# bjo5029/causal-vae

Measured on AMD Instinct MI355X. Metric: training samples/sec on 128^3 vessel volumes (3D CausalVAE train step), higher is better.
Workload: dtype bf16; 1 GPU; 3D vessel CausalVAE train step, 128^3 bf16 volumes (z-scored N(0,1)), batch 4/GPU, Adam lr 0.0001, ELBO = MSE-sum + 2000*MSE-sum(m) + KLD; global_batch=4, per_gpu_batch=4, parallelism=dp1, params=15346957

## Files before the change

causal_vae_amd/_lib.py:

```python
import ctypes as C
import os

import torch

_HERE = os.path.dirname(os.path.abspath(__file__))
LIB_PATH = os.environ.get("CVAE_HIP_LIB") or os.path.join(_HERE, "libcvae_hip.so")

F32, BF16, FP8 = 0, 1, 2
ACT_NONE, ACT_RELU, ACT_SIGMOID, ACT_LEAKY02, ACT_LEAKY001 = 0, 1, 2, 3, 4
_ACT = {None: ACT_NONE, "none": ACT_NONE, "relu": ACT_RELU, "sigmoid": ACT_SIGMOID, "leaky02": ACT_LEAKY02, "leaky001": ACT_LEAKY001}


class CvaeError(RuntimeError):
    pass


if not os.path.exists(LIB_PATH):
    raise ImportError(
        f"{LIB_PATH} is missing: build it with `python -c 'import __graft_entry__ as g; g.build()'` "
        "(or `make -C causal_vae_amd/csrc`).  causal_vae_amd has no CPU / eager fallback.")
lib = C.CDLL(LIB_PATH)

_p, _i64, _i, _f, _sz, _u64 = C.c_void_p, C.c_int64, C.c_int, C.c_float, C.c_size_t, C.c_uint64

# ... 70 lines not shown
    "cvae_softmax_ce_bwd": [_p, _p, _p, _p, _i64, _i64, _p],
    "cvae_uniform_kl_fwd": [_p, _p, _i64, _i64, _p, _sz, _p],
    "cvae_uniform_kl_bwd": [_p, _p, _p, _i64, _i64, _p],
    "cvae_adam_step": [_p, _p, _p, _p, _i64, _f, _f, _f, _f, _f, _f, _p, _p],
    "cvae_adam_multi": [_p, _p, _p, _p, _p, _i, _f, _f, _f, _f, _f, _f, _p, _p, _p],
    "cvae_multi_copy": [_p, _p, _p, _i, _p],
    "cvae_counter_add": [_p, _i, _p],
    "cvae_sqnorm": [_p, _p, _i64, _p, _sz, _p],
    "cvae_sqnorm_multi": [_p, _p, _i, _p, _p, _sz, _p],
    "cvae_weighted_sum": [_p, _p, _i, _p, _p, _i, _p],
    "cvae_scale": [_p, _i64, _p, _p],
    "cvae_clip_coef": [_p, _p, _f, _p],
    "cvae_up2x_supported": [_i64] * 7,
    "cvae_up2x_fwd": [_p, _p] + [_i64] * 7 + [_i, _p],
    "cvae_elbo_up2x_partials": [_i64] * 4,
    "cvae_elbo_up2x_fwd": [_p] * 6 + [_f, _p, _p, _p, _p, _p] + [_i64] * 9 + [_i, _p],
    "cvae_elbo_up2x_bwd": [_p] * 5 + [_f] + [_p] * 5 + [_i64] * 9 + [_i, _p],
    "cvae_conv3_to_k4": [_p, _p, _i64, _i64, _p],
    "cvae_k4_to_conv3_grad": [_p, _p, _i64, _i64, _p],
    "cvae_clamp_fwd": [_p, _p, _f, _f, _i64, _p],
    "cvae_clamp_bwd": [_p, _p, _p, _f, _f, _i64, _p],
    "cvae_bn2d_workspace_bytes": [_i64, _i64],
    "cvae_bn2d_fwd": [_p] * 8 + [_i64, _i64, _f, _f, _i, _i, _i, _p, _sz, _p],
    "cvae_bn2d_bwd": [_p] * 9 + [_i64, _i64, _i, _i, _p, _sz, _p],
    "cvae_fold_bn_conv": [_i] + [_p] * 11 + [_p],
    "cvae_fold_bn_conv_bwd": [_i] + [_p] * 14 + [_p],
    "cvae_vit_tokens": [_p, _i, _p, _p, _p, _i64, _i64, _p],
    "cvae_layernorm256": [_p, _i64, _p, _p, _p, _i64, _f, _i, _p],
    "cvae_token_gemm": [_p, _i64, _p, _p, _p, _i64, _p, _i64, _i64, _i64, _i64, _i, _i, _p],
    "cvae_mhsa_fwd": [_p] * 4 + [_i64] * 9 + [_i, _p],
    "cvae_mhsa_fwd_train": [_p] * 5 + [_i64] * 9 + [_i, _p],
# ... 154 lines not shown
```

causal_vae_amd/csrc/recon_loss.hip:

```cpp
#include "common.h"

namespace {

__device__ __forceinline__ void load4_f32(const float* p, float* o) { const float4 v = *(const float4*)p; o[0] = v.x; o[1] = v.y; o[2] = v.z; o[3] = v.w; }
__device__ __forceinline__ void load4_f32(const bf16* p, float* o) {
    const uint2 v = *(const uint2*)p;
    o[0] = __uint_as_float(v.x << 16); o[1] = __uint_as_float(v.x & 0xffff0000u); o[2] = __uint_as_float(v.y << 16); o[3] = __uint_as_float(v.y & 0xffff0000u);
}

CVAE_TUNABLE(UP2X_STREAM_BYTES, 256 << 20);

__device__ __forceinline__ float2 even_w(int o) { return o == 0 ? make_float2(0.f, 1.f) : make_float2(0.25f, 0.75f); }

#define CVAE_ELBO_TICKET_GROUPS 32
struct ElboFinish {
    unsigned* ticket;
    const float *m_hat, *m, *mu, *logvar;
    float* out4;
    int* bump;
    float gamma;
    int n_m, n_z;
};
struct SmallBwd {
    const float *m_hat, *m, *mu, *logvar;
    float *d_mhat, *dmu, *dlv;
    float gamma;
    int n_m, n_z, main_blocks;
};
template <typename T, int MODE>
__global__ __launch_bounds__(256) void up2x_block_kernel(const T* __restrict__ src, const float* __restrict__ xin, float* __restrict__ dst,
                                                         float* __restrict__ acc_out, const float* __restrict__ gout, float gscale,
                                                         int B, int d, int h, int w, int D, int H, int W, SmallBwd sb, ElboFinish fin) {
    constexpr int J0 = (MODE == 3) ? -1 : 0, NJ = (MODE == 3) ? 10 : 8;
    const bool sdz = D != d;
    const float sw = (float)w / (float)W;
    const int wg = w >> 2, n = B * d * h * wg;
    const int i0 = blockIdx.x * 256 + threadIdx.x, lane = threadIdx.x & 63;
    const bool live = i0 < n;
    const int i = live ? i0 : n - 1;
    float sse = 0.f;
    {
        int r = i;
        const int xg = r % wg; r /= wg;
        const int y = r % h; r /= h;
        const int z = r % d;
        const int b = r / d;
        const int x0 = 4 * xg, ow0 = 8 * xg;
        float4 xa_[2][2], xb_[2][2];
        float xl_[2][2], xr_[2][2];
        if (MODE == 1 || MODE == 3) {
#pragma unroll
            for (int a = 0; a < 2; ++a)
#pragma unroll
                for (int bq = 0; bq < 2; ++bq) {
                    const int od = sdz ? 2 * z + a : z, oh = 2 * y + bq;
                    const size_t rowoff = ((size_t)(b * D + od) * H + oh) * W;
                    xa_[a][bq] = *(const float4*)(xin + rowoff + ow0);
                    xb_[a][bq] = *(const float4*)(xin + rowoff + ow0 + 4);
                    if (MODE == 3) {
                        const float el = xin[rowoff + max(ow0 - 1, 0)], er = xin[rowoff + min(ow0 + 8, W - 1)];
                        const float lft = __shfl_up(xb_[a][bq].w, 1), rgt = __shfl_down(xa_[a][bq].x, 1);
                        xl_[a][bq] = (ow0 > 0) ? (lane > 0 ? lft : el) : 0.f;
                        xr_[a][bq] = (ow0 + 8 < W) ? (lane < 63 ? rgt : er) : 0.f;
                    }
                }
        }
        float P[3][3][NJ];
        const float2 ew0 = even_w(ow0);
#pragma unroll
        for (int zr = 0; zr < 3; ++zr) {
            const int zi = sdz ? min(max(z - 1 + zr, 0), d - 1) : z;
#pragma unroll
            for (int yr = 0; yr < 3; ++yr) {
                const int yi = min(max(y - 1 + yr, 0), h - 1);
                const T* row = src + ((size_t)(b * d + zi) * h + yi) * w;
                float v[6];
                load4_f32(row + x0, v + 1);
                const float el = to_f32(row[max(x0 - 1, 0)]), er = to_f32(row[min(x0 + 4, w - 1)]);
                const float lft = __shfl_up(v[4], 1), rgt = __shfl_down(v[1], 1);
                v[0] = (xg == 0) ? v[1] : (lane > 0 ? lft : el);
                v[5] = (xg == wg - 1) ? v[4] : (lane < 63 ? rgt : er);
#pragma unroll
                for (int j = 0; j < NJ; ++j) {
                    const int jj = J0 + j;
                    if (jj & 1) {
                        const int c = (jj + 1) / 2;
                        P[zr][yr][j] = 0.75f * v[c] + 0.25f * v[c + 1];
                    } else {
                        const int c = jj / 2;
                        const float2 ww = (jj == 0) ? ew0 : make_float2(0.25f, 0.75f);
                        P[zr][yr][j] = ww.x * v[c] + ww.y * v[c + 1];
                    }
                }
            }
        }
        Win4 wx[4];
        if (MODE == 3) {
#pragma unroll
            for (int q = 0; q < 4; ++q) wx[q] = win4<int>(x0 + q, w, W, sw, true);
        }
#pragma unroll
        for (int a = 0; a < 2; ++a) {
            if (!live || (!sdz && a == 1)) break;
            const int od = sdz ? 2 * z + a : z;
            const int zr0 = a;
            const float2 dw = !sdz ? make_float2(1.f, 0.f) : (a == 0 ? even_w(od) : make_float2(0.75f, 0.25f));
#pragma unroll
            for (int bq = 0; bq < 2; ++bq) {
                const int oh = 2 * y + bq;
                const float2 hw = (bq == 0) ? even_w(oh) : make_float2(0.75f, 0.25f);
                float o[NJ];
#pragma unroll
                for (int j = 0; j < NJ; ++j) {
                    const float lo = hw.x * P[zr0][bq][j] + hw.y * P[zr0][bq + 1][j];
                    const float hi = hw.x * P[zr0 + 1][bq][j] + hw.y * P[zr0 + 1][bq + 1][j];
                    o[j] = dw.x * lo + dw.y * hi;
                }
                const size_t rowoff = ((size_t)(b * D + od) * H + oh) * W;
                if (MODE == 0 || MODE == 4) {
                    const f32x4 oa = {o[0], o[1], o[2], o[3]}, ob = {o[4], o[5], o[6], o[7]};
                    if (MODE == 4) {
                        __builtin_nontemporal_store(oa, (f32x4*)(dst + rowoff + ow0));
                        __builtin_nontemporal_store(ob, (f32x4*)(dst + rowoff + ow0 + 4));
                    } else {
                        *(f32x4*)(dst + rowoff + ow0) = oa;
                        *(f32x4*)(dst + rowoff + ow0 + 4) = ob;
                    }
                } else {
                    const float4 xa = xa_[a][bq], xb = xb_[a][bq];
                    const float xv[8] = {xa.x, xa.y, xa.z, xa.w, xb.x, xb.y, xb.z, xb.w};
                    if (MODE == 1) {
#pragma unroll
                        for (int j = 0; j < 8; ++j) { const float df = o[j] - xv[j]; sse += df * df; }
                    } else {
                        float g[10];
                        g[0] = (ow0 > 0) ? o[0] - xl_[a][bq] : 0.f;
#pragma unroll
                        for (int j = 0; j < 8; ++j) { g[1 + j] = o[1 + j] - xv[j]; sse += g[1 + j] * g[1 + j]; }
                        g[9] = (ow0 + 8 < W) ? o[9] - xr_[a][bq] : 0.f;
                        float t1v[4];
#pragma unroll
                        for (int q = 0; q < 4; ++q) {
                            float rs = 0.f;
#pragma unroll
                            for (int c = 0; c < 4; ++c) if (wx[q].w[c] != 0.f) rs += wx[q].w[c] * g[2 * q + c];
                            t1v[q] = rs;
                        }
                        *(float4*)(dst + ((size_t)(b * D + od) * H + oh) * w + x0) = make_float4(t1v[0], t1v[1], t1v[2], t1v[3]);
                    }
                }
            }
        }
    }
    if (MODE == 1 || MODE == 3) {
        __shared__ float red[4];
        __shared__ unsigned is_last;
        sse = wave_sum(sse);
        if ((threadIdx.x & 63) == 0) red[threadIdx.x >> 6] = sse;
        __syncthreads();
        if (!fin.ticket) {
            if (threadIdx.x == 0) acc_out[blockIdx.x] = red[0] + red[1] + red[2] + red[3];
            return;
        }
        if (threadIdx.x == 0) {
            __hip_atomic_store(acc_out + blockIdx.x, red[0] + red[1] + red[2] + red[3], __ATOMIC_RELAXED, __HIP_MEMORY_SCOPE_AGENT);
            asm volatile("s_waitcnt vmcnt(0)" ::: "memory");
            constexpr unsigned G = CVAE_ELBO_TICKET_GROUPS;
            const unsigned grp = blockIdx.x % G, pop = gridDim.x / G + (grp < gridDim.x % G ? 1u : 0u), ngrp = gridDim.x < G ? gridDim.x : G;
            unsigned last = 0u;
            if (__hip_atomic_fetch_add(fin.ticket + 32 * grp, 1u, __ATOMIC_RELAXED, __HIP_MEMORY_SCOPE_AGENT) == pop - 1)
                last = __hip_atomic_fetch_add(fin.ticket + 32 * G, 1u, __ATOMIC_RELAXED, __HIP_MEMORY_SCOPE_AGENT) == ngrp - 1 ? 1u : 0u;
            is_last = last;
        }
        __syncthreads();
        if (!is_last) return;
        __shared__ float fr[3][4];
        float sr = 0.f, sm = 0.f, sk = 0.f;
        for (int i0 = threadIdx.x; i0 < (int)gridDim.x; i0 += 256 * 8) {
            float pv[8];
#pragma unroll
            for (int u = 0; u < 8; ++u) pv[u] = (i0 + 256 * u < (int)gridDim.x) ? __hip_atomic_load(acc_out + i0 + 256 * u, __ATOMIC_RELAXED, __HIP_MEMORY_SCOPE_AGENT) : 0.f;
#pragma unroll
            for (int u = 0; u < 8; ++u) if (i0 + 256 * u < (int)gridDim.x) sr += pv[u];
        }
        for (int i = threadIdx.x; i < fin.n_m; i += 256) { const float df = fin.m_hat[i] - fin.m[i]; sm += df * df; }
        for (int i = threadIdx.x; i < fin.n_z; i += 256) sk += 1.f + fin.logvar[i] - fin.mu[i] * fin.mu[i] - expf(fin.logvar[i]);
        sr = wave_sum(sr); sm = wave_sum(sm); sk = wave_sum(sk);
        if ((threadIdx.x & 63) == 0) { fr[0][threadIdx.x >> 6] = sr; fr[1][threadIdx.x >> 6] = sm; fr[2][threadIdx.x >> 6] = sk; }
        __syncthreads();
        if (threadIdx.x == 0) {
            const float recon = fr[0][0] + fr[0][1] + fr[0][2] + fr[0][3], ml = fr[1][0] + fr[1][1] + fr[1][2] + fr[1][3];
            const float kld = -0.5f * (fr[2][0] + fr[2][1] + fr[2][2] + fr[2][3]);
            fin.out4[0] = recon + fin.gamma * ml + kld; fin.out4[1] = recon; fin.out4[2] = ml; fin.out4[3] = kld;
            if (fin.bump) *fin.bump += 1;
        }
        if (threadIdx.x <= CVAE_ELBO_TICKET_GROUPS) __hip_atomic_store(fin.ticket + 32 * threadIdx.x, 0u, __ATOMIC_RELAXED, __HIP_MEMORY_SCOPE_AGENT);
    }
}

template <typename T, bool NT>
__global__ __launch_bounds__(256) void up2x_tile_kernel(const T* __restrict__ src, float* __restrict__ dst, int d, int h, int w) {
    constexpr int TZ = 2, TY = 8, TX = 64, PZ = TZ + 2, PY = TY + 2, PITCH = TX + 4;
    constexpr int VEC = 16 / sizeof(T), SEGS = TX / VEC;
    __shared__ __attribute__((aligned(16))) float tile[PZ * PY * PITCH];
    const int t = threadIdx.x;
    int blk = blockIdx.x;
    const int xt = blk % (w / TX); blk /= (w / TX);
    const int yt = blk % (h / TY); blk /= (h / TY);
    const int zt = blk % (d / TZ), b = blk / (d / TZ);
    const int x0 = xt * TX, y0 = yt * TY, z0 = zt * TZ;
    const T* sb = src + (size_t)b * d * h * w;
    for (int i = t; i < PZ * PY * SEGS; i += 256) {
// ... 115 lines not shown
    for (int i = threadIdx.x; i < n_z; i += 256) sk += 1.f + logvar[i] - mu[i] * mu[i] - expf(logvar[i]);
    sr = wave_sum(sr); sm = wave_sum(sm); sk = wave_sum(sk);
    if ((threadIdx.x & 63) == 0) { red[0][threadIdx.x >> 6] = sr; red[1][threadIdx.x >> 6] = sm; red[2][threadIdx.x >> 6] = sk; }
    __syncthreads();
    if (threadIdx.x == 0) {
        const float recon = red[0][0] + red[0][1] + red[0][2] + red[0][3], ml = red[1][0] + red[1][1] + red[1][2] + red[1][3];
        const float kld = -0.5f * (red[2][0] + red[2][1] + red[2][2] + red[2][3]);
        out4[0] = recon + gamma * ml + kld; out4[1] = recon; out4[2] = ml; out4[3] = kld;
    }
}

bool up2x_ok(int64_t B, int64_t d, int64_t h, int64_t w, int64_t D, int64_t H, int64_t W) {
    return B > 0 && d > 0 && h > 0 && w > 0 && (D == 2 * d || (D == 1 && d == 1)) && H == 2 * h && W == 2 * w && (w % 4) == 0 && B * D * H * W < (int64_t)1 << 31;
}

}

extern "C" int cvae_up2x_supported(int64_t B, int64_t d, int64_t h, int64_t w, int64_t D, int64_t H, int64_t W) { return up2x_ok(B, d, h, w, D, H, W) ? 1 : 0; }

extern "C" int cvae_up2x_fwd(const void* src, float* dst, int64_t B, int64_t d, int64_t h, int64_t w, int64_t D, int64_t H, int64_t W, int dtype, void* stream) {
    if (!up2x_ok(B, d, h, w, D, H, W)) return CVAE_E_UNSUPPORTED;
    if (!src || !dst) return CVAE_E_NULLPTR;
    const unsigned grid = (unsigned)((B * d * h * (w / 4) + 255) / 256);
    const bool stream_out = B * D * H * W * 4 >= UP2X_STREAM_BYTES;
    if (D == 2 * d && d % 2 == 0 && h % 8 == 0 && w % 64 == 0 && (dtype == CVAE_BF16 || dtype == CVAE_F32)) {
        const dim3 tgrid((unsigned)(B * (d / 2) * (h / 8) * (w / 64)));
        hipStream_t st = (hipStream_t)stream;
#define UP2X_TILE(T, NT) hipLaunchKernelGGL((up2x_tile_kernel<T, NT>), tgrid, dim3(256), 0, st, (const T*)src, dst, (int)d, (int)h, (int)w)
        if (dtype == CVAE_BF16) { if (stream_out) UP2X_TILE(bf16, true); else UP2X_TILE(bf16, false); }
        else { if (stream_out) UP2X_TILE(float, true); else UP2X_TILE(float, false); }
#undef UP2X_TILE
        CVAE_CHECK_LAUNCH();
        return CVAE_OK;
    }
#define UP2X_FWD(T, MODE) hipLaunchKernelGGL((up2x_block_kernel<T, MODE>), dim3(grid), dim3(256), 0, (hipStream_t)stream, (const T*)src, nullptr, dst, nullptr, nullptr, 0.f, (int)B, (int)d, (int)h, (int)w, (int)D, (int)H, (int)W, SmallBwd{}, ElboFinish{})
    if (dtype == CVAE_BF16) { if (stream_out) UP2X_FWD(bf16, 4); else UP2X_FWD(bf16, 0); }
    else if (dtype == CVAE_F32) { if (stream_out) UP2X_FWD(float, 4); else UP2X_FWD(float, 0); }
#undef UP2X_FWD
    else return CVAE_E_DTYPE;
    CVAE_CHECK_LAUNCH();
    return CVAE_OK;
}

extern "C" int64_t cvae_elbo_up2x_partials(int64_t B, int64_t d, int64_t h, int64_t w) { return (B * d * h * (w / 4) + 255) / 256; }

extern "C" int cvae_elbo_up2x_fwd(const void* src, const float* x, const float* m_hat, const float* m, const float* mu, const float* logvar, float gamma,
                                  float* out4, float* partial, float* t1, void* ticket, int* bump, int64_t B, int64_t d, int64_t h, int64_t w, int64_t D, int64_t H, int64_t W,
                                  int64_t n_m, int64_t n_z, int dtype, void* stream) {
    if (!up2x_ok(B, d, h, w, D, H, W) || n_m < 0 || n_z < 0 || n_m > (1 << 24) || n_z > (1 << 24)) return CVAE_E_UNSUPPORTED;
    if (!src || !x || !m_hat || !m || !mu || !logvar || !out4 || !partial) return CVAE_E_NULLPTR;
    if (dtype != CVAE_BF16 && dtype != CVAE_F32) return CVAE_E_DTYPE;
    if (bump && !ticket) return CVAE_E_NULLPTR;
    hipStream_t st = (hipStream_t)stream;
    const unsigned grid = (unsigned)cvae_elbo_up2x_partials(B, d, h, w);
    const ElboFinish fin{(unsigned*)ticket, m_hat, m, mu, logvar, out4, bump, gamma, (int)n_m, (int)n_z};
#define ELBO_FWD(T, MODE) hipLaunchKernelGGL((up2x_block_kernel<T, MODE>), dim3(grid), dim3(256), 0, st, (const T*)src, x, t1, partial, nullptr, 0.f, (int)B, (int)d, (int)h, (int)w, (int)D, (int)H, (int)W, SmallBwd{}, fin)
    if (dtype == CVAE_BF16) { if (t1) ELBO_FWD(bf16, 3); else ELBO_FWD(bf16, 1); }
    else { if (t1) ELBO_FWD(float, 3); else ELBO_FWD(float, 1); }
#undef ELBO_FWD
    CVAE_CHECK_LAUNCH();
    if (!ticket) {
        hipLaunchKernelGGL(elbo_finish_kernel, dim3(1), dim3(256), 0, st, (const float*)partial, (int)grid, m_hat, m, mu, logvar, gamma, out4, (int)n_m, (int)n_z);
        CVAE_CHECK_LAUNCH();
    }
    return CVAE_OK;
}

extern "C" int cvae_elbo_up2x_bwd(const float* t1, const float* m_hat, const float* m, const float* mu, const float* logvar, float gamma, const float* g_loss,
                                  void* dsrc, float* d_mhat, float* dmu, float* dlv, int64_t B, int64_t d, int64_t h, int64_t w, int64_t D, int64_t H, int64_t W,
                                  int64_t n_m, int64_t n_z, int dtype, void* stream) {
    if (!up2x_ok(B, d, h, w, D, H, W) || n_m < 0 || n_z < 0 || n_m > (1 << 24) || n_z > (1 << 24)) return CVAE_E_UNSUPPORTED;
    if (!t1 || !m_hat || !m || !mu || !logvar || !dsrc || !d_mhat || !dmu || !dlv) return CVAE_E_NULLPTR;
    if (dtype != CVAE_BF16 && dtype != CVAE_F32) return CVAE_E_DTYPE;
    hipStream_t st = (hipStream_t)stream;
    const unsigned grid = (unsigned)((B * d * h * (w / 4) + 255) / 256);
    const SmallBwd sb{m_hat, m, mu, logvar, d_mhat, dmu, dlv, gamma, (int)n_m, (int)n_z, (int)grid};
    if (dtype == CVAE_BF16) hipLaunchKernelGGL(up2x_bwd_b_kernel<bf16>, dim3(grid + 1), dim3(256), 0, st, t1, (bf16*)dsrc, g_loss, (int)B, (int)d, (int)h, (int)w, (int)D, (int)H, sb);
// ... 5 lines not shown
```

causal_vae_amd/ops.py:

```python
import ctypes as C_
import math

import torch

from . import _lib as L
from ._lib import lib, check, ptr, stream


_SIDE = {}
FORK_BACKWARD = False
FORK_MAX_POSITIONS = 0
DEFER_JOIN = False
_PENDING = {}


class _Fork:

    def __init__(self, device, positions=None):
        self.main = torch.cuda.current_stream(device)
        key = (device.index if device.index is not None else torch.cuda.current_device())
        self.key = key
        if key not in _SIDE:
            _SIDE[key] = torch.cuda.Stream(device=device)
        on = FORK_BACKWARD and (FORK_MAX_POSITIONS <= 0 or positions is None or positions <= FORK_MAX_POSITIONS)
# ... 1265 lines not shown
    @staticmethod
    def dims(src, x):
        B, d, h, w, Cc = _cl_dims(src)
        sp = tuple(x.shape[2:])
        D, H, W = sp if len(sp) == 3 else (1,) + sp
        return B, d, h, w, Cc, D, H, W

    @staticmethod
    def supported(src, x):
        B, d, h, w, Cc, D, H, W = ElboUp2x.dims(src, x)
        return (Cc == 1 and x.shape[0] == B and x.shape[1] == 1 and x.dtype == torch.float32 and bool(lib.cvae_up2x_supported(B, d, h, w, D, H, W)))

    _tickets = {}
    IN_LAUNCH_FINISH = __import__("os").environ.get("CVAE_ELBO_TWO_LAUNCH") != "1"

    @staticmethod
    def forward(ctx, src, x, m_hat, m, mu, logvar, gamma, bump=None):
        L.require_gpu(src, x, m_hat, m, mu, logvar)
        src = src.contiguous()
        x, m_hat, m, mu, logvar = (t.contiguous().float() for t in (x, m_hat, m, mu, logvar))
        if m_hat.shape != m.shape or mu.shape != logvar.shape:
            raise RuntimeError(f"The size of tensor a {tuple(m_hat.shape)} must match the size of tensor b {tuple(m.shape)}")
        B, d, h, w, Cc, D, H, W = ElboUp2x.dims(src, x)
        buf = torch.empty(4 + lib.cvae_elbo_up2x_partials(B, d, h, w), dtype=torch.float32, device=x.device)
        t1 = torch.empty(B * D * H * w, dtype=torch.float32, device=x.device) if any(ctx.needs_input_grad[i] for i in (0, 2, 4, 5)) else None
        ticket = None
        if ElboUp2x.IN_LAUNCH_FINISH:
            ticket = ElboUp2x._tickets.get(x.device)
            if ticket is None:
                ticket = ElboUp2x._tickets[x.device] = torch.zeros(33 * 32, dtype=torch.int32, device=x.device)
        check(lib.cvae_elbo_up2x_fwd(ptr(src), ptr(x), ptr(m_hat), ptr(m), ptr(mu), ptr(logvar), float(gamma), ptr(buf), buf.data_ptr() + 16, ptr(t1), ptr(ticket),
                                     ptr(bump) if ticket is not None else None, B, d, h, w, D, H, W, m.numel(), mu.numel(), L.dtype_code(src.dtype), stream()), "elbo_up2x_fwd")
        if bump is not None and ticket is None:
            check(lib.cvae_counter_add(ptr(bump), 1, stream()), "counter_add")
        ctx.save_for_backward(src, x, m_hat, m, mu, logvar, t1)
        ctx.gamma = float(gamma)
        ctx.set_materialize_grads(False)
        return buf[0], buf[1], buf[2], buf[3]

    @staticmethod
    def backward(ctx, g_loss, g_recon, g_m, g_kld):
        src, x, m_hat, m, mu, logvar, t1 = ctx.saved_tensors
        if g_recon is not None or g_m is not None or g_kld is not None:
            raise L.CvaeError("ElboUp2x back-propagates the total loss only; for a single term use loss_function on the model's recon_x")
        if g_loss is None:
            return None, None, None, None, None, None, None, None
        B, d, h, w, Cc, D, H, W = ElboUp2x.dims(src, x)
# ... 1047 lines not shown
```

include/cvae_hip.h:

```cpp
#ifndef CVAE_HIP_H
#define CVAE_HIP_H
#include <stddef.h>
#include <stdint.h>

#ifdef __cplusplus
extern "C" {
#endif

#define CVAE_OK             0
#define CVAE_E_BADSHAPE    (-1)
#define CVAE_E_DTYPE       (-2)
#define CVAE_E_UNSUPPORTED (-3)
#define CVAE_E_WORKSPACE   (-4)
#define CVAE_E_LAUNCH      (-5)
#define CVAE_E_NULLPTR     (-6)

#define CVAE_F32  0
#define CVAE_BF16 1
#define CVAE_FP8  2

#define CVAE_ACT_NONE    0
#define CVAE_ACT_RELU    1
#define CVAE_ACT_SIGMOID 2
#define CVAE_ACT_LEAKY02 3
// ... 42 lines not shown
                  float out8_inv_scale, void* amax_slots, int64_t B, int64_t sd, int64_t sh, int64_t sw, int64_t Cs, int64_t ld, int64_t lh, int64_t lw, int64_t Cl,
                  int nd, int act, void* workspace, size_t workspace_bytes, int xpair, void* relu_bits_out, void* stream);
int cvae_conv_up_c1_fp8in(const void* S8, const float* w, const float* bias, void* L, float in_scale, int64_t B, int64_t sd, int64_t sh, int64_t sw, int64_t Cs, int nd, int act,
                          void* stream);
int cvae_conv_down_image_f8(const void* L, int l_dtype, const float* w, const float* bias, void* S, void* S8, const float* inv_scale_dev, void* amax_slots,
                            void* relu_bits_out, int64_t B, int64_t sd, int64_t sh, int64_t sw, int64_t Cs, int64_t ld, int64_t lh, int64_t lw, int nd, int act,
                            void* stream);
int cvae_fp8_scale_update(void* amax_slots, float* scale, float* inv_scale, int n, float headroom, const int* layer_in, const int* layer_w, const int* layer_out,
                          int n_layers, float* dscale, void* ticket, void* stream);
int cvae_up2x_supported(int64_t B, int64_t d, int64_t h, int64_t w, int64_t D, int64_t H, int64_t W);
int cvae_up2x_fwd(const void* src, float* dst, int64_t B, int64_t d, int64_t h, int64_t w, int64_t D, int64_t H, int64_t W, int dtype, void* stream);
#define CVAE_ELBO_TICKET_WORDS (33 * 32)
int64_t cvae_elbo_up2x_partials(int64_t B, int64_t d, int64_t h, int64_t w);
int cvae_elbo_up2x_fwd(const void* src, const float* x, const float* m_hat, const float* m, const float* mu, const float* logvar, float gamma,
                       float* out4, float* partial, float* t1, void* ticket, int* bump, int64_t B, int64_t d, int64_t h, int64_t w, int64_t D, int64_t H, int64_t W,
                       int64_t n_m, int64_t n_z, int dtype, void* stream);
int cvae_elbo_up2x_bwd(const float* t1, const float* m_hat, const float* m, const float* mu, const float* logvar, float gamma, const float* g_loss,
                       void* dsrc, float* d_mhat, float* dmu, float* dlv, int64_t B, int64_t d, int64_t h, int64_t w, int64_t D, int64_t H, int64_t W,
                       int64_t n_m, int64_t n_z, int dtype, void* stream);

int cvae_conv3_to_k4(const float* w3 , float* k4 , int64_t Cout, int64_t Cin, void* stream);
int cvae_k4_to_conv3_grad(const float* dk4, float* dw3, int64_t Cout, int64_t Cin, void* stream);
int cvae_clamp_fwd(const float* x, float* y, float lo, float hi, int64_t n, void* stream);
int cvae_clamp_bwd(const float* x, const float* g, float* dx, float lo, float hi, int64_t n, void* stream);
size_t cvae_bn2d_workspace_bytes(int64_t P, int64_t C);
int cvae_bn2d_fwd(const void* x, const float* gamma, const float* beta, void* y, float* mean, float* rstd, float* running_mean, float* running_var,
                  int64_t P, int64_t C, float momentum, float eps, int training, int act, int dtype, void* workspace, size_t workspace_bytes, void* stream);
int cvae_bn2d_bwd(const void* x, const void* dy, const void* y, const float* gamma, const float* mean, const float* rstd, void* dx, float* dgamma,
                  float* dbeta, int64_t P, int64_t C, int act, int dtype, void* workspace, size_t workspace_bytes, void* stream);

#define CVAE_FOLD_CONV_K4   0
// ... 225 lines not shown
```

Before: 5234 samples/s.

## Add persistent LDS-tiled ELBO upsample-loss forward kernel with halo reuse

Adds a persistent, grid-capped kernel for the fused trilinear-2x-upsample plus reconstruction-SSE forward. Each workgroup stages source rows with halos in LDS and walks units of rows, so neighbouring rows reuse loaded data instead of re-reading the 3x3 stencil from global memory. It also refactors the per-item math into a shared helper with explicit FMAs and moves the last-block finish logic into a shared function. The cost is more code paths, an added API argument, LDS pressure, and ablation knobs left in the hot kernels.

After: 5293 samples/s, median of 6. +1.1%, better.

```diff
diff --git a/causal_vae_amd/_lib.py b/causal_vae_amd/_lib.py
--- a/causal_vae_amd/_lib.py
+++ b/causal_vae_amd/_lib.py
@@ -108,7 +108,8 @@
     "cvae_up2x_supported": [_i64] * 7,
     "cvae_up2x_fwd": [_p, _p] + [_i64] * 7 + [_i, _p],
     "cvae_elbo_up2x_partials": [_i64] * 4,
-    "cvae_elbo_up2x_fwd": [_p] * 6 + [_f, _p, _p, _p, _p, _p] + [_i64] * 9 + [_i, _p],
+    "cvae_elbo_up2x_tiled": [_i64] * 7,
+    "cvae_elbo_up2x_fwd": [_p] * 6 + [_f, _p, _p, _p, _p, _p] + [_i64] * 9 + [_i, _p, _i],
     "cvae_elbo_up2x_bwd": [_p] * 5 + [_f] + [_p] * 5 + [_i64] * 9 + [_i, _p],
     "cvae_conv3_to_k4": [_p, _p, _i64, _i64, _p],
     "cvae_k4_to_conv3_grad": [_p, _p, _i64, _i64, _p],
diff --git a/causal_vae_amd/csrc/recon_loss.hip b/causal_vae_amd/csrc/recon_loss.hip
--- a/causal_vae_amd/csrc/recon_loss.hip
+++ b/causal_vae_amd/csrc/recon_loss.hip
@@ -9,6 +9,8 @@
 }
 
 CVAE_TUNABLE(UP2X_STREAM_BYTES, 256 << 20);
+CVAE_TUNABLE(ELBO_ABLATE, 0);
+CVAE_TUNABLE(ELBO_TILE_WGS, 512);
 
 __device__ __forceinline__ float2 even_w(int o) { return o == 0 ? make_float2(0.f, 1.f) : make_float2(0.25f, 0.75f); }
 
@@ -20,6 +22,7 @@
     int* bump;
     float gamma;
     int n_m, n_z;
+    int n_partial;
 };
 struct SmallBwd {
     const float *m_hat, *m, *mu, *logvar;
@@ -27,11 +30,137 @@
     float gamma;
     int n_m, n_z, main_blocks;
 };
+
+__device__ __forceinline__ Win4 win4_exact2x(int i, int in) {
+    Win4 r;
+    r.j0 = 2 * i - 1;
+    r.w[0] = i > 0 ? 0.25f : 0.f;
+    r.w[1] = i > 0 ? 0.75f : 1.f;
+    r.w[2] = i < in - 1 ? 0.75f : 1.f;
+    r.w[3] = i < in - 1 ? 0.25f : 0.f;
+    return r;
+}
+
+template <int MODE, typename SDZ, typename LoadV, typename GetX, typename RowDone>
+__device__ __forceinline__ float up2x_item(bool live, SDZ sdz, int z, int y, int x0, int w, int W, float sw, LoadV&& load_v, GetX&& get_x, RowDone&& row_done) {
+#pragma clang fp contract(off)
+    constexpr int J0 = (MODE == 3) ? -1 : 0, NJ = (MODE == 3) ? 10 : 8;
+    const int ow0 = 2 * x0;
+    float sse = 0.f;
+    Win4 wx[4];
+    if (MODE == 3) {
+#pragma unroll
+        for (int q = 0; q < 4; ++q) wx[q] = win4_exact2x(x0 + q, w);
+    }
+    float HL[2][2][NJ];
+    const float2 ew0 = even_w(ow0);
+#pragma unroll
+    for (int zr = 0; zr < 3; ++zr) {
+        float P[3][NJ];
+#pragma unroll
+        for (int yr = 0; yr < 3; ++yr) {
+            float v[6];
+            load_v(zr, yr, v);
+#pragma unroll
+            for (int j = 0; j < NJ; ++j) {
+                const int jj = J0 + j;
+                if (jj & 1) {
+                    const int c = (jj + 1) / 2;
+                    P[yr][j] = fmaf(0.75f, v[c], 0.25f * v[c + 1]);
+                } else {
+                    const int c = jj / 2;
+                    const float2 ww = (jj == 0) ? ew0 : make_float2(0.25f, 0.75f);
+                    P[yr][j] = fmaf(ww.x, v[c], ww.y * v[c + 1]);
+                }
+            }
+        }
+#pragma unroll
+        for (int bq = 0; bq < 2; ++bq) {
+            const float2 hw = (bq == 0) ? even_w(2 * y) : make_float2(0.75f, 0.25f);
+#pragma unroll
+            for (int j = 0; j < NJ; ++j) HL[zr & 1][bq][j] = fmaf(hw.x, P[bq][j], hw.y * P[bq + 1][j]);
+        }
+        const int a = zr - 1;
+        if (zr == 0 || !live || (!sdz && a == 1)) continue;
+        const int od = sdz ? 2 * z + a : z;
+        const float2 dw = !sdz ? make_float2(1.f, 0.f) : (a == 0 ? even_w(od) : make_float2(0.75f, 0.25f));
+#pragma unroll
+        for (int bq = 0; bq < 2; ++bq) {
+            const int oh = 2 * y + bq;
+            float o[NJ];
+#pragma unroll
+            for (int j = 0; j < NJ; ++j) o[j] = fmaf(dw.x, HL[a & 1][bq][j], dw.y * HL[(a + 1) & 1][bq][j]);
+            if (MODE == 0 || MODE == 4) {
+                row_done(a, bq, od, oh, o);
+            } else {
+                float xv[8], xl = 0.f, xr = 0.f;
+                get_x(a, bq, xv, xl, xr);
+                if (MODE == 1) {
+#pragma unroll
+                    for (int j = 0; j < 8; ++j) { const float df = o[j] - xv[j]; sse = fmaf(df, df, sse); }
+                    row_done(a, bq, od, oh, (const float*)nullptr);
+                } else {
+                    float g[10];
+                    g[0] = (ow0 > 0) ? o[0] - xl : 0.f;
+#pragma unroll
+                    for (int j = 0; j < 8; ++j) { g[1 + j] = o[1 + j] - xv[j]; sse = fmaf(g[1 + j], g[1 + j], sse); }
+                    g[9] = (ow0 + 8 < W) ? o[9] - xr : 0.f;
+                    float t1v[4];
+#pragma unroll
+                    for (int q = 0; q < 4; ++q) {
+                        float rs = 0.f;
+#pragma unroll
+                        for (int c = 0; c < 4; ++c) if (wx[q].w[c] != 0.f) rs = fmaf(wx[q].w[c], g[2 * q + c], rs);
+                        t1v[q] = rs;
+                    }
+                    row_done(a, bq, od, oh, t1v);
+                }
+            }
+        }
+    }
+    return sse;
+}
+
+__device__ __forceinline__ void elbo_arrive_and_finish(const float* acc_out, const ElboFinish& fin) {
+    __shared__ unsigned is_last;
+    if (threadIdx.x == 0) {
+        asm volatile("s_waitcnt vmcnt(0)" ::: "memory");
+        constexpr unsigned G = CVAE_ELBO_TICKET_GROUPS;
+        const unsigned grp = blockIdx.x % G, pop = gridDim.x / G + (grp < gridDim.x % G ? 1u : 0u), ngrp = gridDim.x < G ? gridDim.x : G;
+        unsigned last = 0u;
+        if (__hip_atomic_fetch_add(fin.ticket + 32 * grp, 1u, __ATOMIC_RELAXED, __HIP_MEMORY_SCOPE_AGENT) == pop - 1)
+            last = __hip_atomic_fetch_add(fin.ticket + 32 * G, 1u, __ATOMIC_RELAXED, __HIP_MEMORY_SCOPE_AGENT) == ngrp - 1 ? 1u : 0u;
+        is_last = last;
+    }
+    __syncthreads();
+    if (!is_last) return;
+    __shared__ float fr[3][4];
+    float sr = 0.f, sm = 0.f, sk = 0.f;
+    for (int i0 = threadIdx.x; i0 < fin.n_partial; i0 += 256 * 8) {
+        float pv[8];
+#pragma unroll
+        for (int u = 0; u < 8; ++u) pv[u] = (i0 + 256 * u < fin.n_partial) ? __hip_atomic_load(acc_out + i0 + 256 * u, __ATOMIC_RELAXED, __HIP_MEMORY_SCOPE_AGENT) : 0.f;
+#pragma unroll
+        for (int u = 0; u < 8; ++u) if (i0 + 256 * u < fin.n_partial) sr += pv[u];
+    }
+    for (int i = threadIdx.x; i < fin.n_m; i += 256) { const float df = fin.m_hat[i] - fin.m[i]; sm += df * df; }
+    for (int i = threadIdx.x; i < fin.n_z; i += 256) sk += 1.f + fin.logvar[i] - fin.mu[i] * fin.mu[i] - expf(fin.logvar[i]);
+    sr = wave_sum(sr); sm = wave_sum(sm); sk = wave_sum(sk);
+    if ((threadIdx.x & 63) == 0) { fr[0][threadIdx.x >> 6] = sr; fr[1][threadIdx.x >> 6] = sm; fr[2][threadIdx.x >> 6] = sk; }
+    __syncthreads();
+    if (threadIdx.x == 0) {
+        const float recon = fr[0][0] + fr[0][1] + fr[0][2] + fr[0][3], ml = fr[1][0] + fr[1][1] + fr[1][2] + fr[1][3];
+        const float kld = -0.5f * (fr[2][0] + fr[2][1] + fr[2][2] + fr[2][3]);
+        fin.out4[0] = recon + fin.gamma * ml + kld; fin.out4[1] = recon; fin.out4[2] = ml; fin.out4[3] = kld;
+        if (fin.bump) *fin.bump += 1;
+    }
+    if (threadIdx.x <= CVAE_ELBO_TICKET_GROUPS) __hip_atomic_store(fin.ticket + 32 * threadIdx.x, 0u, __ATOMIC_RELAXED, __HIP_MEMORY_SCOPE_AGENT);
+}
+
 template <typename T, int MODE>
 __global__ __launch_bounds__(256) void up2x_block_kernel(const T* __restrict__ src, const float* __restrict__ xin, float* __restrict__ dst,
                                                          float* __restrict__ acc_out, const float* __restrict__ gout, float gscale,
                                                          int B, int d, int h, int w, int D, int H, int W, SmallBwd sb, ElboFinish fin) {
-    constexpr int J0 = (MODE == 3) ? -1 : 0, NJ = (MODE == 3) ? 10 : 8;
     const bool sdz = D != d;
     const float sw = (float)w / (float)W;
     const int wg = w >> 2, n = B * d * h * wg;
@@ -55,6 +184,7 @@
                 for (int bq = 0; bq < 2; ++bq) {
                     const int od = sdz ? 2 * z + a : z, oh = 2 * y + bq;
                     const size_t rowoff = ((size_t)(b * D + od) * H + oh) * W;
+                    if (ELBO_ABLATE & 2) { xa_[a][bq] = xb_[a][bq] = make_float4(gscale, gscale, gscale, gscale); xl_[a][bq] = xr_[a][bq] = gscale; continue; }
                     xa_[a][bq] = *(const float4*)(xin + rowoff + ow0);
                     xb_[a][bq] = *(const float4*)(xin + rowoff + ow0 + 4);
                     if (MODE == 3) {
@@ -65,137 +195,160 @@
                     }
                 }
         }
-        float P[3][3][NJ];
-        const float2 ew0 = even_w(ow0);
-#pragma unroll
-        for (int zr = 0; zr < 3; ++zr) {
-            const int zi = sdz ? min(max(z - 1 + zr, 0), d - 1) : z;
-#pragma unroll
-            for (int yr = 0; yr < 3; ++yr) {
-                const int yi = min(max(y - 1 + yr, 0), h - 1);
-                const T* row = src + ((size_t)(b * d + zi) * h + yi) * w;
-                float v[6];
-                load4_f32(row + x0, v + 1);
-                const float el = to_f32(row[max(x0 - 1, 0)]), er = to_f32(row[min(x0 + 4, w - 1)]);
-                const float lft = __shfl_up(v[4], 1), rgt = __shfl_down(v[1], 1);
-                v[0] = (xg == 0) ? v[1] : (lane > 0 ? lft : el);
-                v[5] = (xg == wg - 1) ? v[4] : (lane < 63 ? rgt : er);
-#pragma unroll
-                for (int j = 0; j < NJ; ++j) {
-                    const int jj = J0 + j;
-                    if (jj & 1) {
-                        const int c = (jj + 1) / 2;
-                        P[zr][yr][j] = 0.75f * v[c] + 0.25f * v[c + 1];
-                    } else {
-                        const int c = jj / 2;
-                        const float2 ww = (jj == 0) ? ew0 : make_float2(0.25f, 0.75f);
-                        P[zr][yr][j] = ww.x * v[c] + ww.y * v[c + 1];
-                    }
+        const auto load_v = [&](int zr, int yr, float* v) {
+            const int zi = sdz ? min(max(z - 1 + zr, 0), d - 1) : z, yi = min(max(y - 1 + yr, 0), h - 1);
+            const T* row = src + ((size_t)(b * d + zi) * h + yi) * w;
+            if (ELBO_ABLATE & 8) { for (int q = 0; q < 6; ++q) v[q] = gscale + (float)(zi + yi + q); return; }
+            load4_f32(row + x0, v + 1);
+            const float el = to_f32(row[max(x0 - 1, 0)]), er = to_f32(row[min(x0 + 4, w - 1)]);
+            const float lft = __shfl_up(v[4], 1), rgt = __shfl_down(v[1], 1);
+            v[0] = (xg == 0) ? v[1] : (lane > 0 ? lft : el);
+            v[5] = (xg == wg - 1) ? v[4] : (lane < 63 ? rgt : er);
+        };
+        const auto get_x = [&](int a, int bq, float* xv, float& xl, float& xr) {
+            const float4 xa = xa_[a][bq], xb = xb_[a][bq];
+            xv[0] = xa.x; xv[1] = xa.y; xv[2] = xa.z; xv[3] = xa.w; xv[4] = xb.x; xv[5] = xb.y; xv[6] = xb.z; xv[7] = xb.w;
+            if (MODE == 3) { xl = xl_[a][bq]; xr = xr_[a][bq]; }
+        };
+        const auto row_done = [&](int a, int bq, int od, int oh, const float* r) {
+            if (MODE == 0 || MODE == 4) {
+                const size_t rowoff = ((size_t)(b * D + od) * H + oh) * W;
+                const f32x4 oa = {r[0], r[1], r[2], r[3]}, ob = {r[4], r[5], r[6], r[7]};
+                if (MODE == 4) {
+                    __builtin_nontemporal_store(oa, (f32x4*)(dst + rowoff + ow0));
+                    __builtin_nontemporal_store(ob, (f32x4*)(dst + rowoff + ow0 + 4));
+                } else {
+                    *(f32x4*)(dst + rowoff + ow0) = oa;
+                    *(f32x4*)(dst + rowoff + ow0 + 4) = ob;
                 }
+            } else if (MODE == 3) {
+                if ((ELBO_ABLATE & 1) && gscale == 0.f) return;
+                *(float4*)(dst + ((size_t)(b * D + od) * H + oh) * w + x0) = make_float4(r[0], r[1], r[2], r[3]);
             }
-        }
-        Win4 wx[4];
-        if (MODE == 3) {
-#pragma unroll
-            for (int q = 0; q < 4; ++q) wx[q] = win4<int>(x0 + q, w, W, sw, true);
-        }
-#pragma unroll
-        for (int a = 0; a < 2; ++a) {
-            if (!live || (!sdz && a == 1)) break;
-            const int od = sdz ? 2 * z + a : z;
-            const int zr0 = a;
-            const float2 dw = !sdz ? make_float2(1.f, 0.f) : (a == 0 ? even_w(od) : make_float2(0.75f, 0.25f));
-#pragma unroll
-            for (int bq = 0; bq < 2; ++bq) {
-                const int oh = 2 * y + bq;
-                const float2 hw = (bq == 0) ? even_w(oh) : make_float2(0.75f, 0.25f);
-                float o[NJ];
-#pragma unroll
-                for (int j = 0; j < NJ; ++j) {
-                    const float lo = hw.x * P[zr0][bq][j] + hw.y * P[zr0][bq + 1][j];
-                    const float hi = hw.x * P[zr0 + 1][bq][j] + hw.y * P[zr0 + 1][bq + 1][j];
-                    o[j] = dw.x * lo + dw.y * hi;
-                }
-                const size_t rowoff = ((size_t)(b * D + od) * H + oh) * W;
-                if (MODE == 0 || MODE == 4) {
-                    const f32x4 oa = {o[0], o[1], o[2], o[3]}, ob = {o[4], o[5], o[6], o[7]};
-                    if (MODE == 4) {
-                        __builtin_nontemporal_store(oa, (f32x4*)(dst + rowoff + ow0));
-                        __builtin_nontemporal_store(ob, (f32x4*)(dst + rowoff + ow0 + 4));
-                    } else {
-                        *(f32x4*)(dst + rowoff + ow0) = oa;
-                        *(f32x4*)(dst + rowoff + ow0 + 4) = ob;
-                    }
-                } else {
-                    const float4 xa = xa_[a][bq], xb = xb_[a][bq];
-                    const float xv[8] = {xa.x, xa.y, xa.z, xa.w, xb.x, xb.y, xb.z, xb.w};
-                    if (MODE == 1) {
-#pragma unroll
-                        for (int j = 0; j < 8; ++j) { const float df = o[j] - xv[j]; sse += df * df; }
-                    } else {
-                        float g[10];
-                        g[0] = (ow0 > 0) ? o[0] - xl_[a][bq] : 0.f;
-#pragma unroll
-                        for (int j = 0; j < 8; ++j) { g[1 + j] = o[1 + j] - xv[j]; sse += g[1 + j] * g[1 + j]; }
-                        g[9] = (ow0 + 8 < W) ? o[9] - xr_[a][bq] : 0.f;
-                        float t1v[4];
-#pragma unroll
-                        for (int q = 0; q < 4; ++q) {
-                            float rs = 0.f;
-#pragma unroll
-                            for (int c = 0; c < 4; ++c) if (wx[q].w[c] != 0.f) rs += wx[q].w[c] * g[2 * q + c];
-                            t1v[q] = rs;
-                        }
-                        *(float4*)(dst + ((size_t)(b * D + od) * H + oh) * w + x0) = make_float4(t1v[0], t1v[1], t1v[2], t1v[3]);
-                    }
-                }
-            }
-        }
+        };
+        sse = up2x_item<MODE>(live, sdz, z, y, x0, w, W, sw, load_v, get_x, row_done);
     }
     if (MODE == 1 || MODE == 3) {
         __shared__ float red[4];
-        __shared__ unsigned is_last;
         sse = wave_sum(sse);
         if ((threadIdx.x & 63) == 0) red[threadIdx.x >> 6] = sse;
         __syncthreads();
-        if (!fin.ticket) {
+        if (!fin.ticket || (ELBO_ABLATE & 4)) {
             if (threadIdx.x == 0) acc_out[blockIdx.x] = red[0] + red[1] + red[2] + red[3];
             return;
         }
-        if (threadIdx.x == 0) {
-            __hip_atomic_store(acc_out + blockIdx.x, red[0] + red[1] + red[2] + red[3], __ATOMIC_RELAXED, __HIP_MEMORY_SCOPE_AGENT);
-            asm volatile("s_waitcnt vmcnt(0)" ::: "memory");
-            constexpr unsigned G = CVAE_ELBO_TICKET_GROUPS;
-            const unsigned grp = blockIdx.x % G, pop = gridDim.x / G + (grp < gridDim.x % G ? 1u : 0u), ngrp = gridDim.x < G ? gridDim.x : G;
-            unsigned last = 0u;
-            if (__hip_atomic_fetch_add(fin.ticket + 32 * grp, 1u, __ATOMIC_RELAXED, __HIP_MEMORY_SCOPE_AGENT) == pop - 1)
-                last = __hip_atomic_fetch_add(fin.ticket + 32 * G, 1u, __ATOMIC_RELAXED, __HIP_MEMORY_SCOPE_AGENT) == ngrp - 1 ? 1u : 0u;
-            is_last = last;
-        }
+        if (threadIdx.x == 0) __hip_atomic_store(acc_out + blockIdx.x, red[0] + red[1] + red[2] + red[3], __ATOMIC_RELAXED, __HIP_MEMORY_SCOPE_AGENT);
+        elbo_arrive_and_finish(acc_out, fin);
+    }
+}
+
+template <typename T, int MODE, int NV, bool SDZ>
+__global__ __launch_bounds__(256) void elbo_tile_kernel(const T* __restrict__ src, const float* __restrict__ xin, float* __restrict__ t1,
+                                                        float* __restrict__ partial, int units, int d, int h, int w, int D, ElboFinish fin) {
+    typedef typename std::conditional<sizeof(T) == 2, uint2, float4>::type Raw;
+    extern __shared__ __attribute__((aligned(16))) float elbo_tile[];
+    __shared__ float red[4];
+    const int t = threadIdx.x, lane = t & 63;
+    constexpr std::bool_constant<SDZ> sdz{};
+    const int H = 2 * h, W = 2 * w, wg = w >> 2, lg = 31 - __clz(wg), R = 256 >> lg, PY = R + 2, PITCH = w + 4;
+    const float sw = (float)w / (float)W;
+    const int xg = t & (wg - 1), yl = t >> lg, x0 = 4 * xg, ow0 = 8 * xg;
+    const unsigned lx = 2 * yl * W + ow0, lt = 2 * yl * w + x0;
+    struct Unit { int b, z, y0; };
+    const auto unit_of = [&](int u) { const int row0 = u * R, pl = row0 / h; return Unit{pl / d, pl % d, row0 - pl * h}; };
+    const auto halo_row = [&](int k) { return min((k - 3) * R + yl, 5); };
+    const auto issue_src = [&](const Unit& un, Raw (&sv)[NV]) {
+#pragma unroll
+        for (int k = 0; k < NV; ++k) {
+            const int e = halo_row(k), pz = k < 3 ? k : e >> 1;
+            const int zi = sdz ? min(max(un.z - 1 + pz, 0), d - 1) : un.z;
+            const int yi = k < 3 ? un.y0 + yl : ((e & 1) ? min(un.y0 + R, h - 1) : max(un.y0 - 1, 0));
+            sv[k] = *(const Raw*)(src + (unsigned)(((un.b * d + zi) * h + yi) * w + x0));
+        }
+    };
+    const auto stage_src = [&](const Raw (&sv)[NV]) {
+#pragma unroll
+        for (int k = 0; k < NV; ++k) {
+            const int e = (k - 3) * R + yl;
+            if (k >= 3 && e >= 6) continue;
+            const int row = k < 3 ? k * PY + 1 + yl : (e >> 1) * PY + ((e & 1) ? R + 1 : 0);
+            float v[4];
+            if constexpr (sizeof(T) == 2) {
+                v[0] = __uint_as_float(sv[k].x << 16); v[1] = __uint_as_float(sv[k].x & 0xffff0000u);
+                v[2] = __uint_as_float(sv[k].y << 16); v[3] = __uint_as_float(sv[k].y & 0xffff0000u);
+            } else {
+                v[0] = sv[k].x; v[1] = sv[k].y; v[2] = sv[k].z; v[3] = sv[k].w;
+            }
+            float* o = elbo_tile + row * PITCH + 1 + x0;
+#pragma unroll
+            for (int q = 0; q < 4; ++q) o[q] = v[q];
+            if (xg == 0) o[-1] = v[0];
+            if (xg == wg - 1) o[4] = v[3];
+        }
+    };
+    f32x4 xa_[2][2], xb_[2][2];
+    const auto issue_x = [&](const Unit& un, int a, int bq, bool real) {
+        const int od = sdz ? 2 * un.z + a : un.z, oh0 = 2 * un.y0 + bq;
+        const float* row = xin + (real ? ((size_t)(un.b * D + od) * H + oh0) * W : (size_t)0);
+        xa_[a][bq] = *(const f32x4*)(row + lx);
+        xb_[a][bq] = *(const f32x4*)(row + lx + 4);
+    };
+    int u = blockIdx.x;
+    Unit cu = unit_of(u);
+    Raw sv[NV];
+    issue_src(cu, sv);
+#pragma unroll
+    for (int a = 0; a < 2; ++a)
+#pragma unroll
+        for (int bq = 0; bq < 2; ++bq) if (sdz || a == 0) issue_x(cu, a, bq, true);
+    for (;;) {
+        stage_src(sv);
         __syncthreads();
-        if (!is_last) return;
-        __shared__ float fr[3][4];
-        float sr = 0.f, sm = 0.f, sk = 0.f;
-        for (int i0 = threadIdx.x; i0 < (int)gridDim.x; i0 += 256 * 8) {
-            float pv[8];
-#pragma unroll
-            for (int u = 0; u < 8; ++u) pv[u] = (i0 + 256 * u < (int)gridDim.x) ? __hip_atomic_load(acc_out + i0 + 256 * u, __ATOMIC_RELAXED, __HIP_MEMORY_SCOPE_AGENT) : 0.f;
-#pragma unroll
-            for (int u = 0; u < 8; ++u) if (i0 + 256 * u < (int)gridDim.x) sr += pv[u];
-        }
-        for (int i = threadIdx.x; i < fin.n_m; i += 256) { const float df = fin.m_hat[i] - fin.m[i]; sm += df * df; }
-        for (int i = threadIdx.x; i < fin.n_z; i += 256) sk += 1.f + fin.logvar[i] - fin.mu[i] * fin.mu[i] - expf(fin.logvar[i]);
-        sr = wave_sum(sr); sm = wave_sum(sm); sk = wave_sum(sk);
-        if ((threadIdx.x & 63) == 0) { fr[0][threadIdx.x >> 6] = sr; fr[1][threadIdx.x >> 6] = sm; fr[2][threadIdx.x >> 6] = sk; }
+        const int un = u + (int)gridDim.x;
+        const bool more = un < units;
+        const Unit nu = unit_of(more ? un : u);
+        issue_src(nu, sv);
+        const int y = cu.y0 + yl;
+        const auto load_v = [&](int zr, int yr, float* v) {
+            const float* rp = elbo_tile + (zr * PY + yl + yr) * PITCH + x0;
+            const float4 va = *(const float4*)rp;
+            const float2 vb = *(const float2*)(rp + 4);
+            v[0] = va.x; v[1] = va.y; v[2] = va.z; v[3] = va.w; v[4] = vb.x; v[5] = vb.y;
+        };
+        const auto get_x = [&](int a, int bq, float* xv, float& xl, float& xr) {
+            const f32x4 xa = xa_[a][bq], xb = xb_[a][bq];
+#pragma unroll
+            for (int q = 0; q < 4; ++q) { xv[q] = xa[q]; xv[4 + q] = xb[q]; }
+            if (MODE == 3) {
+                float el = 0.f, er = 0.f;
+                if (NV > 4 && wg > 64) {
+                    const int od = sdz ? 2 * cu.z + a : cu.z, oh = 2 * y + bq;
+                    const float* row = xin + ((size_t)(cu.b * D + od) * H + oh) * W;
+                    el = row[max(ow0 - 1, 0)]; er = row[min(ow0 + 8, W - 1)];
+                }
+                const float lft = __shfl_up(xb[3], 1), rgt = __shfl_down(xa[0], 1);
+                xl = (ow0 > 0) ? (lane > 0 ? lft : el) : 0.f;
+                xr = (ow0 + 8 < W) ? (lane < 63 ? rgt : er) : 0.f;
+            }
+        };
+        const auto row_done = [&](int a, int bq, int od, int oh, const float* r) {
+            if (MODE == 3) *(float4*)(t1 + ((size_t)(cu.b * D + od) * H + 2 * cu.y0 + bq) * w + lt) = make_float4(r[0], r[1], r[2], r[3]);
+            __builtin_amdgcn_sched_barrier(0);
+            issue_x(nu, a, bq, more);
+        };
+        float sse = up2x_item<MODE>(true, sdz, cu.z, y, x0, w, W, sw, load_v, get_x, row_done);
+        sse = wave_sum(sse);
+        if (lane == 0) red[t >> 6] = sse;
         __syncthreads();
-        if (threadIdx.x == 0) {
-            const float recon = fr[0][0] + fr[0][1] + fr[0][2] + fr[0][3], ml = fr[1][0] + fr[1][1] + fr[1][2] + fr[1][3];
-            const float kld = -0.5f * (fr[2][0] + fr[2][1] + fr[2][2] + fr[2][3]);
-            fin.out4[0] = recon + fin.gamma * ml + kld; fin.out4[1] = recon; fin.out4[2] = ml; fin.out4[3] = kld;
-            if (fin.bump) *fin.bump += 1;
-        }
-        if (threadIdx.x <= CVAE_ELBO_TICKET_GROUPS) __hip_atomic_store(fin.ticket + 32 * threadIdx.x, 0u, __ATOMIC_RELAXED, __HIP_MEMORY_SCOPE_AGENT);
-    }
+        if (t == 0) {
+            const float s = red[0] + red[1] + red[2] + red[3];
+            if (fin.ticket) __hip_atomic_store(partial + u, s, __ATOMIC_RELAXED, __HIP_MEMORY_SCOPE_AGENT);
+            else partial[u] = s;
+        }
+        if (!more) break;
+        u = un; cu = nu;
+    }
+    if (fin.ticket) elbo_arrive_and_finish(partial, fin);
 }
 
 template <typename T, bool NT>
@@ -341,6 +494,19 @@
     return B > 0 && d > 0 && h > 0 && w > 0 && (D == 2 * d || (D == 1 && d == 1)) && H == 2 * h && W == 2 * w && (w % 4) == 0 && B * D * H * W < (int64_t)1 << 31;
 }
 
+bool elbo_tiled_ok(int64_t B, int64_t d, int64_t h, int64_t w, int64_t D, int64_t H, int64_t W) {
+    if (!up2x_ok(B, d, h, w, D, H, W)) return false;
+    const int64_t wg = w / 4;
+    return wg <= 256 && 256 % wg == 0 && h % (256 / wg) == 0;
+}
+size_t elbo_tile_lds(int64_t w) { return (size_t)3 * (256 / (w / 4) + 2) * (w + 4) * sizeof(float); }
+
+template <typename T, int MODE, int NV, bool SDZ>
+void elbo_tile_launch(unsigned grid, hipStream_t st, const void* src, const float* x, float* t1, float* partial, int units, int64_t d, int64_t h, int64_t w, int64_t D,
+                      const ElboFinish& fin) {
+    hipLaunchKernelGGL((elbo_tile_kernel<T, MODE, NV, SDZ>), dim3(grid), dim3(256), elbo_tile_lds(w), st, (const T*)src, x, t1, partial, units, (int)d, (int)h, (int)w, (int)D, fin);
+}
+
 }
 
 extern "C" int cvae_up2x_supported(int64_t B, int64_t d, int64_t h, int64_t w, int64_t D, int64_t H, int64_t W) { return up2x_ok(B, d, h, w, D, H, W) ? 1 : 0; }
@@ -371,23 +537,45 @@
 
 extern "C" int64_t cvae_elbo_up2x_partials(int64_t B, int64_t d, int64_t h, int64_t w) { return (B * d * h * (w / 4) + 255) / 256; }
 
+extern "C" int cvae_elbo_up2x_tiled(int64_t B, int64_t d, int64_t h, int64_t w, int64_t D, int64_t H, int64_t W) { return elbo_tiled_ok(B, d, h, w, D, H, W) ? 1 : 0; }
+
 extern "C" int cvae_elbo_up2x_fwd(const void* src, const float* x, const float* m_hat, const float* m, const float* mu, const float* logvar, float gamma,
                                   float* out4, float* partial, float* t1, void* ticket, int* bump, int64_t B, int64_t d, int64_t h, int64_t w, int64_t D, int64_t H, int64_t W,
-                                  int64_t n_m, int64_t n_z, int dtype, void* stream) {
-    if (!up2x_ok(B, d, h, w, D, H, W) || n_m < 0 || n_z < 0 || n_m > (1 << 24) || n_z > (1 << 24)) return CVAE_E_UNSUPPORTED;
+                                  int64_t n_m, int64_t n_z, int dtype, void* stream, int form) {
+    if (!up2x_ok(B, d, h, w, D, H, W) || n_m < 0 || n_z < 0 || n_m > (1 << 24) || n_z > (1 << 24) || form < -1) return CVAE_E_UNSUPPORTED;
+    const bool tileable = elbo_tiled_ok(B, d, h, w, D, H, W);
+    if (form >= 1 && !tileable) return CVAE_E_UNSUPPORTED;
     if (!src || !x || !m_hat || !m || !mu || !logvar || !out4 || !partial) return CVAE_E_NULLPTR;
     if (dtype != CVAE_BF16 && dtype != CVAE_F32) return CVAE_E_DTYPE;
     if (bump && !ticket) return CVAE_E_NULLPTR;
     hipStream_t st = (hipStream_t)stream;
-    const unsigned grid = (unsigned)cvae_elbo_up2x_partials(B, d, h, w);
-    const ElboFinish fin{(unsigned*)ticket, m_hat, m, mu, logvar, out4, bump, gamma, (int)n_m, (int)n_z};
-#define ELBO_FWD(T, MODE) hipLaunchKernelGGL((up2x_block_kernel<T, MODE>), dim3(grid), dim3(256), 0, st, (const T*)src, x, t1, partial, nullptr, 0.f, (int)B, (int)d, (int)h, (int)w, (int)D, (int)H, (int)W, SmallBwd{}, fin)
-    if (dtype == CVAE_BF16) { if (t1) ELBO_FWD(bf16, 3); else ELBO_FWD(bf16, 1); }
-    else { if (t1) ELBO_FWD(float, 3); else ELBO_FWD(float, 1); }
+    const unsigned n_partial = (unsigned)cvae_elbo_up2x_partials(B, d, h, w);
+    const ElboFinish fin{(unsigned*)ticket, m_hat, m, mu, logvar, out4, bump, gamma, (int)n_m, (int)n_z, (int)n_partial};
+    if (form != 0 && tileable) {
+        const unsigned cap = form >= 1 ? (unsigned)form : (unsigned)ELBO_TILE_WGS, grid = n_partial < cap ? n_partial : cap;
+        with_dtype(dtype, [&](auto tv) {
+            using T = decltype(tv);
+            with_bool(256 / (w / 4) >= 8, [&](auto few) {
+                constexpr int NV = decltype(few)::value ? 4 : 9;
+                with_bool(D != d, [&](auto sdz) {
+                    constexpr bool SDZ = decltype(sdz)::value;
+                    if (t1) elbo_tile_launch<T, 3, NV, SDZ>(grid, st, src, x, t1, partial, (int)n_partial, d, h, w, D, fin);
+                    else elbo_tile_launch<T, 1, NV, SDZ>(grid, st, src, x, t1, partial, (int)n_partial, d, h, w, D, fin);
+                    return 0;
+                });
+                return 0;
+            });
+            return 0;
+        });
+    } else {
+#define ELBO_FWD(T, MODE) hipLaunchKernelGGL((up2x_block_kernel<T, MODE>), dim3(n_partial), dim3(256), 0, st, (const T*)src, x, t1, partial, nullptr, 0.f, (int)B, (int)d, (int)h, (int)w, (int)D, (int)H, (int)W, SmallBwd{}, fin)
+        if (dtype == CVAE_BF16) { if (t1) ELBO_FWD(bf16, 3); else ELBO_FWD(bf16, 1); }
+        else { if (t1) ELBO_FWD(float, 3); else ELBO_FWD(float, 1); }
 #undef ELBO_FWD
+    }
     CVAE_CHECK_LAUNCH();
     if (!ticket) {
-        hipLaunchKernelGGL(elbo_finish_kernel, dim3(1), dim3(256), 0, st, (const float*)partial, (int)grid, m_hat, m, mu, logvar, gamma, out4, (int)n_m, (int)n_z);
+        hipLaunchKernelGGL(elbo_finish_kernel, dim3(1), dim3(256), 0, st, (const float*)partial, (int)n_partial, m_hat, m, mu, logvar, gamma, out4, (int)n_m, (int)n_z);
         CVAE_CHECK_LAUNCH();
     }
     return CVAE_OK;
diff --git a/causal_vae_amd/ops.py b/causal_vae_amd/ops.py
--- a/causal_vae_amd/ops.py
+++ b/causal_vae_amd/ops.py
@@ -1303,6 +1303,8 @@
     _tickets = {}
     IN_LAUNCH_FINISH = __import__("os").environ.get("CVAE_ELBO_TWO_LAUNCH") != "1"
 
+    FORM = -1
+
     @staticmethod
     def forward(ctx, src, x, m_hat, m, mu, logvar, gamma, bump=None):
         L.require_gpu(src, x, m_hat, m, mu, logvar)
@@ -1319,7 +1321,7 @@
             if ticket is None:
                 ticket = ElboUp2x._tickets[x.device] = torch.zeros(33 * 32, dtype=torch.int32, device=x.device)
         check(lib.cvae_elbo_up2x_fwd(ptr(src), ptr(x), ptr(m_hat), ptr(m), ptr(mu), ptr(logvar), float(gamma), ptr(buf), buf.data_ptr() + 16, ptr(t1), ptr(ticket),
-                                     ptr(bump) if ticket is not None else None, B, d, h, w, D, H, W, m.numel(), mu.numel(), L.dtype_code(src.dtype), stream()), "elbo_up2x_fwd")
+                                     ptr(bump) if ticket is not None else None, B, d, h, w, D, H, W, m.numel(), mu.numel(), L.dtype_code(src.dtype), stream(), ElboUp2x.FORM), "elbo_up2x_fwd")
         if bump is not None and ticket is None:
             check(lib.cvae_counter_add(ptr(bump), 1, stream()), "counter_add")
         ctx.save_for_backward(src, x, m_hat, m, mu, logvar, t1)
diff --git a/include/cvae_hip.h b/include/cvae_hip.h
--- a/include/cvae_hip.h
+++ b/include/cvae_hip.h
@@ -80,7 +80,8 @@
 int64_t cvae_elbo_up2x_partials(int64_t B, int64_t d, int64_t h, int64_t w);
 int cvae_elbo_up2x_fwd(const void* src, const float* x, const float* m_hat, const float* m, const float* mu, const float* logvar, float gamma,
                        float* out4, float* partial, float* t1, void* ticket, int* bump, int64_t B, int64_t d, int64_t h, int64_t w, int64_t D, int64_t H, int64_t W,
-                       int64_t n_m, int64_t n_z, int dtype, void* stream);
+                       int64_t n_m, int64_t n_z, int dtype, void* stream, int form);
+int cvae_elbo_up2x_tiled(int64_t B, int64_t d, int64_t h, int64_t w, int64_t D, int64_t H, int64_t W);
 int cvae_elbo_up2x_bwd(const float* t1, const float* m_hat, const float* m, const float* mu, const float* logvar, float gamma, const float* g_loss,
                        void* dsrc, float* d_mhat, float* dmu, float* dlv, int64_t B, int64_t d, int64_t h, int64_t w, int64_t D, int64_t H, int64_t W,
                        int64_t n_m, int64_t n_z, int dtype, void* stream);
```
